# KorAP/Datok

Measured on AMD Instinct MI355X. Metric: input MB/s tokenized, tokenizer_de.matok, higher is better.
Workload: dtype u32 table cells, u8 symbol codes; 1 GPU; tokenizer_de.matok, 4096 equal-length 4096 B synthetic German docs per batch (BASELINE.json configs[1]); table_layout=matrix: state-major fused u32 cells, docs_per_gpu=4096, doc_bytes=4096, parallelism=documents sharded over 1 GPU(s), no data-path collective, batches_in_flight=3, inputs=one per batch in flight (generator seeds 2, 3, 4 on rank 0)

## Files before the change

datok_amd/_lib.py:

```python
import ctypes as C
import os
import subprocess

_HERE = os.path.dirname(os.path.abspath(__file__))
LIB_PATH = os.environ.get("DATOK_GPU_LIB") or os.path.join(_HERE, "libdatok_gpu.so")

OK, E_IO, E_FORMAT, E_NO_DEVICE, E_HIP, E_ARG, E_MODEL, E_CAPACITY, E_STATE, E_NOMEM = 0, -1, -2, -3, -4, -5, -6, -7, -8, -9
ST_WINDOW_OVERFLOW, ST_EMPTY_TEXT, ST_BAD_MODEL, ST_IRREGULAR, ST_STEP_LIMIT, ST_INTERNAL = 1, 2, 4, 8, 16, 32
ST_BAD_OFFSET = 64

EXPORTS = [
    "dtk_device_count", "dtk_set_device", "dtk_strerror", "dtk_last_hip_error",
    "dtk_model_load", "dtk_model_load_mem", "dtk_model_free", "dtk_model_type", "dtk_model_get_info",
    "dtk_model_info_mem",
    "dtk_batch_create", "dtk_batch_free", "dtk_batch_set_input", "dtk_batch_set_input_device",
    "dtk_batch_run", "dtk_batch_sync", "dtk_batch_stream", "dtk_batch_totals",
    "dtk_batch_set_profiling", "dtk_batch_stage_ms", "dtk_batch_set_chunking", "dtk_batch_set_warm_extend",
    "dtk_batch_result_device", "dtk_batch_result_host", "dtk_transduce", "dtk_free",
    "dtk_foma_to_matok", "dtk_foma_to_datok", "dtk_transduce_replay", "dtk_batch_render_device", "dtk_batch_render_host",
    "dtk_batch_status_host", "dtk_transduce_release", "dtk_transduce_result",
    "dtk_pipeline_create", "dtk_pipeline_free", "dtk_pipeline_set_chunking", "dtk_pipeline_run",
    "dtk_pinned_alloc", "dtk_pinned_free",
    "dtk_batch_set_result_fields", "dtk_batch_download_begin", "dtk_pipeline_set_result_fields",
    "dtk_batch_set_download_stream", "dtk_batch_download_stream", "dtk_batch_done", "dtk_batch_set_streams",
    "dtk_debug_configure",
    "dtk_multi_create", "dtk_multi_free", "dtk_multi_type", "dtk_multi_set_result_fields", "dtk_multi_set_chunking", "dtk_multi_run",
]


class ModelInfo(C.Structure):
    _fields_ = [("kind", C.c_int32), ("epsilon", C.c_int32), ("unknown", C.c_int32),
                ("identity", C.c_int32), ("final_state", C.c_int32), ("sigma_count", C.c_int32),
                ("state_count", C.c_uint32), ("array_len", C.c_uint64),
                ("n_eps_states", C.c_uint32), ("max_eps_chain", C.c_uint32),
                ("entry_bytes", C.c_uint32), ("device_bytes", C.c_uint64),
                ("unknown_used", C.c_uint32), ("dense_states", C.c_uint32),
                ("stream_codes", C.c_uint32)]


class Totals(C.Structure):
    _fields_ = [("n_docs", C.c_uint32), ("n_bytes", C.c_uint64), ("n_tokens", C.c_uint64),
                ("n_sent", C.c_uint64), ("n_texts", C.c_uint64), ("n_flagged", C.c_uint64),
                ("walk_steps", C.c_uint64), ("n_lanes", C.c_uint32), ("chunk_bytes", C.c_uint32),
                ("repair_rounds", C.c_uint32)]


class ResultView(C.Structure):
    _fields_ = [("tok_off", C.c_void_p), ("sent_off", C.c_void_p), ("text_off", C.c_void_p),
# ... 95 lines not shown
    L.dtk_foma_to_matok.restype = C.c_int
    L.dtk_foma_to_datok.argtypes = [vp, C.c_size_t, C.POINTER(vp), C.POINTER(C.c_size_t)]
    L.dtk_foma_to_datok.restype = C.c_int
    L.dtk_free.argtypes = [vp]
    L.dtk_free.restype = None
    L.dtk_pipeline_create.argtypes = [u64, u32, u32, C.POINTER(vp)]
    L.dtk_pipeline_free.argtypes = [vp]
    L.dtk_pipeline_free.restype = None
    L.dtk_pipeline_set_chunking.argtypes = [vp, u32, u32]
    L.dtk_pipeline_run.argtypes = [vp, vp, vp, vp, u32, u32, SLICE_FN, vp]
    L.dtk_multi_create.argtypes = [C.c_char_p, C.POINTER(C.c_int), u32, u64, u32, u32, C.POINTER(vp)]
    L.dtk_multi_free.argtypes = [vp]
    L.dtk_multi_free.restype = None
    L.dtk_multi_type.argtypes = [vp]
    L.dtk_multi_type.restype = C.c_char_p
    L.dtk_multi_set_result_fields.argtypes = [vp, u32]
    L.dtk_multi_set_chunking.argtypes = [vp, u32, u32]
    L.dtk_multi_run.argtypes = [vp, vp, vp, u32, u32, SLICE_FN, vp]
    L.dtk_pinned_alloc.restype = vp
    L.dtk_pinned_alloc.argtypes = [sz]
    L.dtk_pinned_free.argtypes = [vp]
    L.dtk_pinned_free.restype = None
    L.dtk_debug_configure.argtypes = [C.c_char_p, C.c_char_p]
    for k, v in os.environ.items():
        if k.startswith("DATOK_") and k not in ("DATOK_GPU_LIB", "DATOK_GATHER_TIMEOUT"):
            L.dtk_debug_configure(k.encode(), v.encode())
    _lib = L
    return L


def check(code, what=""):
    if code != OK:
        raise DatokGpuError(code, what)
```

datok_amd/csrc/dtk_batch.cpp:

```cpp
#include <algorithm>
#include <cstdio>
#include <cstring>

#include "dtk_host.h"

int pin_fit(dtk_batch::PinBuf &pb, size_t n) {
  if (n <= pb.cap && pb.p) return DTK_OK;
  if (pb.p) HIP_TRY(hipHostFree(pb.p));
  pb.p = nullptr; pb.cap = 0;
  const size_t cap = std::max<size_t>(n + n / 4, 256);
  HIP_TRY(hipHostMalloc(&pb.p, cap, hipHostMallocDefault));
  pb.cap = cap;
  return DTK_OK;
}

static int alloc_outputs(dtk_batch *b, uint64_t tok, uint64_t sent, uint64_t text) {
  auto grow = [&](auto *&p, uint64_t n) -> int {
    if (p) HIP_TRY(hipFree(p));
    p = nullptr;
    HIP_TRY(hipMalloc((void **)&p, std::max<uint64_t>(n, 4) * 4));
    return DTK_OK;
  };
  int rc;
  if (tok > b->tok_cap) {
// ... 23 lines not shown
  if (dtk_device_count() <= 0) return DTK_E_NO_DEVICE;
  dtk_batch *b = new dtk_batch();
  b->max_bytes = max_bytes;
  b->max_docs = max_docs;
  auto fail = [&](int rc) { dtk_batch_free(b); return rc; };
#define B_TRY(call)                                                  \
  do {                                                               \
    hipError_t e_ = (call);                                          \
    if (e_ != hipSuccess) return fail(hip_fail(e_, #call));          \
  } while (0)
  B_TRY(hipGetDevice(&b->device));
  B_TRY(hipStreamCreateWithFlags(&b->stream, hipStreamNonBlocking));
  if (g_dbg.round_limit >= 0) b->round_limit = (uint32_t)g_dbg.round_limit;
  const uint64_t pad = 256;
  B_TRY(hipMalloc((void **)&b->d_text_own, max_bytes + pad));
  B_TRY(hipMalloc((void **)&b->d_off_own, ((uint64_t)max_docs + 1) * 8));
  B_TRY(hipMalloc((void **)&b->d_sym, (max_bytes + pad) * 2));
  B_TRY(hipMalloc((void **)&b->d_rsbits, (max_bytes + pad) / 8 + 64));
  B_TRY(hipMalloc((void **)&b->d_bits, (EVB_KINDS * ((max_bytes + max_docs) / 32 + 8) + 8) * 4));
  b->acc_bytes = DTK_TOTALS_BYTES + 3 * ((uint64_t)max_docs + 1) * 8 + 4 * (uint64_t)max_docs * 4 + 64;
  B_TRY(hipMalloc((void **)&b->d_acc, b->acc_bytes));
  B_TRY(hipMalloc((void **)&b->d_redo, (uint64_t)max_docs * 4));
  B_TRY(hipMalloc((void **)&b->d_blk_doc, (max_bytes / DTK_SYM_BLOCK_BYTES + 3) * 4));

  B_TRY(hipMalloc((void **)&b->d_chunk_off, ((uint64_t)max_docs + 1) * 4));
  B_TRY(hipMalloc((void **)&b->d_big_docs, ((uint64_t)max_docs + 1) * 4));
  B_TRY(hipMalloc((void **)&b->d_csr, 3 * ((uint64_t)max_docs + 1) * 8));
  b->d_tok_off = b->d_csr; b->d_sent_off = b->d_csr + ((uint64_t)max_docs + 1); b->d_text_off = b->d_csr + 2 * ((uint64_t)max_docs + 1);
  B_TRY(hipMalloc((void **)&b->d_doc_ns, ((uint64_t)max_docs + 1) * 4));
  B_TRY(hipMalloc((void **)&b->d_scan_ws, ((uint64_t)max_docs / 2048 + 2) * 4 * 8));
  B_TRY(hipMalloc((void **)&b->d_out_off, ((uint64_t)max_docs + 1) * 8));

  B_TRY(hipHostMalloc((void **)&b->h_totals, DTK_TOTALS_BYTES, hipHostMallocDefault));
  B_TRY(hipHostMalloc((void **)&b->h_off_pin, ((uint64_t)max_docs + 1) * 8, hipHostMallocDefault));
#undef B_TRY
  int rc = alloc_outputs(b, max_bytes / 3 + max_docs + 16, max_bytes / 8 + 2ull * max_docs + 16,
                         max_bytes / 64 + 2ull * max_docs + 16);
  if (rc != DTK_OK) return fail(rc);
  *out = b;
  return DTK_OK;
}

extern "C" void dtk_batch_free(dtk_batch *b) {
  if (!b) return;
  if (b->stream) (void)hipStreamSynchronize(b->stream);
  if (b->up_stream) (void)hipStreamSynchronize(b->up_stream);
  if (b->ev_up) (void)hipEventDestroy(b->ev_up);
  if (b->dl_begun && !b->dl_waited) (void)hipEventSynchronize(b->ev_dl);
  if (b->dl_stream && b->dl_own) (void)hipStreamDestroy(b->dl_stream);
  if (b->ev_ran) (void)hipEventDestroy(b->ev_ran);
  if (b->ev_dl) (void)hipEventDestroy(b->ev_dl);
  for (auto &pb : b->pin)
    if (pb.p) (void)hipHostFree(pb.p);
  if (b->h_plan.p) (void)hipHostFree(b->h_plan.p);
  void *ptrs[] = {b->d_text_own, b->d_off_own, b->d_sym, b->d_rsbits, b->d_bits, b->d_acc, b->d_redo, b->d_chunk_off, b->d_blk_doc, b->d_big_docs,
                  b->d_lane_doc, b->d_lane_cnt, b->d_lane_start, b->d_lane_end, b->d_lane_plan,
                  b->d_seg_tab, b->d_seg_sum, b->d_seg_in,
                  b->d_csr, b->d_rstart, b->d_rend, b->d_sent,
                  b->d_bstart, b->d_bend, b->d_ttok, b->d_tsent,
                  b->d_sbefore, b->d_ts_end, b->d_doc_ns, b->d_scan_ws, b->d_rws, b->d_out_off, b->d_out,
                  b->d_exact_ids, b->d_exact_cnt, b->d_exact_off, b->d_calls, b->d_r16};
  for (void *p : ptrs)
    if (p) (void)hipFree(p);
  if (b->h_totals) (void)hipHostFree(b->h_totals);
  if (b->h_off_pin) (void)hipHostFree(b->h_off_pin);
  for (hipEvent_t e : b->ev)
    if (e) (void)hipEventDestroy(e);
  if (b->stream && b->stream_own) (void)hipStreamDestroy(b->stream);
  delete b;
}

extern "C" void *dtk_batch_stream(dtk_batch *b) { return b ? (void *)b->stream : nullptr; }

static int wait_ran(dtk_batch *b) {
  if (b->stream_own) HIP_TRY(hipStreamSynchronize(b->stream));
  else if (b->ev_ran_valid) HIP_TRY(hipEventSynchronize(b->ev_ran));
  return DTK_OK;
}
// ... 310 lines not shown
    b->d_tok_off = b->d_csr; b->d_sent_off = b->d_csr + (nd + 1); b->d_text_off = b->d_csr + 2 * (nd + 1);
    b->d_totals = (uint64_t *)q; q += DTK_TOTALS_BYTES;
    b->d_tok_cnt = (uint64_t *)q; q += (nd + 1) * 8;
    b->d_sent_cnt = (uint64_t *)q; q += (nd + 1) * 8;
    b->d_text_cnt = (uint64_t *)q; q += (nd + 1) * 8;
    b->d_status = (uint32_t *)q; q += nd * 4;
    b->d_first_bad = (uint32_t *)q; q += nd * 4;
    b->d_fail_lane = (uint32_t *)q; q += nd * 4;
    b->d_doc_tail = (uint32_t *)q; q += nd * 4;
    const size_t acc_used = ((size_t)(q - b->d_acc) + 15) & ~(size_t)15;
    b->bit_words = (uint32_t)(((b->total + nd) / 32 + 8) & ~(uint64_t)3);
    const bool fold = b->total > 0;
    fold_acc = fold && b->acc_primed && acc_used / 16 < 0xFFFFFFFFull && !g_dbg.clear_kernel;
    if (!fold_acc) {
      if (dtk_launch_clear2(b->d_acc, acc_used, b->d_bits, fold ? 0 : (size_t)EVB_KINDS * b->bit_words * 4, s))
        return hip_fail(hipGetLastError(), "clear");
      b->acc_primed = true;
    }
    acc_bytes = acc_used;
  }
  STAGE(1);
  if (dtk_launch_symbolize(b->d_text, b->d_off, b->n_docs, b->total, &m->sig, b->d_sym,
                           b->d_text == b->d_text_own, b->d_blk_doc, (unsigned long long *)(b->d_totals + 6), b->d_rsbits,
                           b->d_bits, b->bit_words, fold_acc ? b->d_acc : nullptr, acc_bytes, ++b->epoch, s))
    return hip_fail(hipGetLastError(), "symbolize");
  STAGE(2);
  DtkWalkArgs w = walk_args(b);
  bool fix_in_scan = false;
  DtkSpecArgs sp_first{};
  if (b->chunk == 0) {
    STAGE(3); STAGE(4);
    if (dtk_launch_walk(&m->tab, &w, s)) return hip_fail(hipGetLastError(), "walk");
    STAGE(5); STAGE(6); STAGE(7);
  } else {
    DtkSpecArgs sp = spec_args(b, false);
    sp_first = sp;
    uint32_t *nb = (uint32_t *)(b->d_totals + 8);
    const bool split = g_dbg.split_start != 0 || sp.lds_words == 0;
    b->dev_rounds = g_dbg.dev_rounds >= 0 ? (uint32_t)g_dbg.dev_rounds : (b->expect_repairs ? 2u : 0u);
    if (b->dev_rounds > 3u) b->dev_rounds = 3u;
    fix_in_scan = b->n_docs <= 8192u && b->dev_rounds == 0;
#define SPEC(stage)                                                                               \
  do {                                                                                            \
    if (dtk_launch_spec(&m->tab, &w, &sp, stage, cmp_mask_of(m), b->d_redo, nb, s))               \
      return hip_fail(hipGetLastError(), "speculative walk");                                     \
  } while (0)
    if (split) {
// ... 51 lines not shown
  if (e != hipSuccess) (void)hipGetLastError();
  return e == hipSuccess ? 1 : 0;
}

extern "C" int dtk_batch_set_profiling(dtk_batch *b, int enable) {
  if (!b) return DTK_E_ARG;
  if (enable && !b->ev[0])
    for (auto &e : b->ev) HIP_TRY(hipEventCreate(&e));
  b->profiling = enable != 0;
  return DTK_OK;
}

extern "C" int dtk_batch_stage_ms(dtk_batch *b, float ms[DTK_N_STAGES]) {
  if (!b || !ms) return DTK_E_ARG;
  if (!b->ran || !b->profiling) return DTK_E_STATE;
  HIP_TRY(hipStreamSynchronize(b->stream));
  for (int i = 0; i < DTK_N_STAGES; i++) HIP_TRY(hipEventElapsedTime(&ms[i], b->ev[i], b->ev[i + 1]));
  return DTK_OK;
}

extern "C" int dtk_batch_sync(dtk_batch *b) {
  if (!b) return DTK_E_ARG;
  return wait_own(b);
}

static int run_exact(dtk_batch *b) {
  const dtk_model *m = b->last_model;
  hipStream_t s = b->stream;
  const uint32_t nd = b->n_docs;
  std::vector<uint32_t> st(nd);
  HIP_TRY(hipMemcpy(st.data(), b->d_status, (size_t)nd * 4, hipMemcpyDeviceToHost));
  for (uint32_t d = 0; d < nd; d++)
    if (st[d] & ST_IRREGULAR) b->h_exact_ids.push_back(d);
  const uint32_t n = (uint32_t)b->h_exact_ids.size();
  if (n == 0) return DTK_OK;
  if (n > b->exact_cap) {
    void *old[] = {b->d_exact_ids, b->d_exact_cnt, b->d_exact_off};
    for (void *p : old)
      if (p) HIP_TRY(hipFree(p));
    b->d_exact_ids = b->d_exact_cnt = nullptr; b->d_exact_off = nullptr; b->exact_cap = 0;
    const uint64_t cap = (uint64_t)n + n / 4 + 16;
    HIP_TRY(hipMalloc((void **)&b->d_exact_ids, cap * 4));
    HIP_TRY(hipMalloc((void **)&b->d_exact_cnt, cap * 4));
    HIP_TRY(hipMalloc((void **)&b->d_exact_off, (cap + 1) * 8));
    b->exact_cap = (uint32_t)cap;
  }
// ... 161 lines not shown
```

datok_amd/csrc/dtk_host.h:

```cpp
#pragma once
#include <hip/hip_runtime.h>

#include <string>
#include <type_traits>
#include <vector>

#include "../../include/datok_gpu.h"
#include "dtk_internal.h"

#pragma GCC visibility push(hidden)


int hip_fail(hipError_t e, const char *what);
#define HIP_TRY(call)                                   \
  do {                                                  \
    hipError_t e_ = (call);                             \
    if (e_ != hipSuccess) return hip_fail(e_, #call);   \
  } while (0)

struct DtkDebug {
  int sym16 = 0;
  int force_wide = 0;
  int file_columns = 0;
  int no_fused = 0;
  int wide_fused = 0;
  int no_dense = 0;
  int small_max = -1;
  int lds_bits = 1;
  int split_start = 0;
  int dev_rounds = -1;
  int compact_full = 0;
  int clear_kernel = 0;
  int round_limit = -1;
  int debug_repair = 0;
};
extern DtkDebug g_dbg;


struct dtk_model {
  int kind = 0;
  int epsilon = 0, unknown = 0, identity = 0, final_state = 0, sigma_count = 0;
  uint32_t state_count = 0;
  std::vector<uint16_t> col;
  uint32_t dense_states = 0;
  uint64_t array_len = 0;
  uint32_t n_eps_states = 0, max_eps_chain = 0, unknown_used = 0;
  uint64_t device_bytes = 0;
  int device = 0;
  bool host_only = false;
  std::vector<uint32_t> sigma_runes;
  std::vector<uint16_t> sigma_syms;
  uint16_t ascii[256];
  void *d_tab = nullptr;
  uint16_t *d_ascii = nullptr;
  uint32_t *d_runes = nullptr;
  uint16_t *d_syms = nullptr;
  void *d_codes = nullptr;
// ... 22 lines not shown
  uint16_t *d_sym = nullptr;
  uint32_t *d_rsbits = nullptr;
  uint32_t *d_bits = nullptr;
  uint32_t bit_words = 0;
  uint32_t *d_doc_tail = nullptr;
  uint8_t *d_acc = nullptr;
  uint64_t acc_bytes = 0;
  uint32_t *d_status = nullptr;
  std::vector<uint64_t> h_doc_off;
  uint32_t cfg_chunk = 0xFFFFFFFFu;
  uint32_t cfg_extend = 240;
  uint32_t cfg_warm = 8;
  uint32_t chunk = 0;
  bool plan_valid = false;
  uint32_t n_lanes = 0, lane_cap = 0;
  uint32_t *d_lane_doc = nullptr, *d_chunk_off = nullptr, *d_redo = nullptr;
  uint32_t *d_seg_tab = nullptr;
  DtkSegSum *d_seg_sum = nullptr;
  DtkSegIn *d_seg_in = nullptr;
  uint32_t n_segs = 0, seg_cap = 0;
  bool long_docs = false;
  uint32_t max_doc_lanes = 0;
  uint32_t *d_blk_doc = nullptr;
  uint32_t small_max = 0, n_big = 0;
  uint32_t *d_big_docs = nullptr;
  uint32_t *d_first_bad = nullptr, *d_fail_lane = nullptr;
  DtkLaneCount *d_lane_cnt = nullptr;
  DtkLaneState *d_lane_start = nullptr, *d_lane_end = nullptr;
  DtkLanePlan *d_lane_plan = nullptr;
  uint32_t repair_rounds = 0;
  const dtk_model *last_model = nullptr;
  uint32_t last_flags = 0;
  uint64_t *d_csr = nullptr;
  uint64_t *d_tok_off = nullptr, *d_sent_off = nullptr, *d_text_off = nullptr;
  uint64_t *d_tok_cnt = nullptr, *d_sent_cnt = nullptr, *d_text_cnt = nullptr;
  uint64_t *d_scan_ws = nullptr;
  uint64_t *d_totals = nullptr;
  uint32_t dev_rounds = 0;
  bool expect_repairs = false;
  uint32_t round_limit = 0xFFFFFFFFu;
  bool acc_primed = false;
  uint64_t epoch = 0;
  bool expect_eot = false;
  bool ran_full = false;
  uint64_t *h_totals = nullptr;
  uint64_t *h_off_pin = nullptr;
// ... 80 lines not shown
```

datok_amd/csrc/dtk_internal.h:

```cpp
#pragma once
#include <stddef.h>
#include <stdint.h>

#define DTK_FIRSTBIT 0x80000000u
#define DTK_SECONDBIT 0x40000000u
#define DTK_RESTBIT 0x3fffffffu
#define DTK_EOT 4u
#define DTK_WINDOW 1024u
#define DTK_WINDOW_BYTES 4104u

#define DTK_SYM_MASK 0x7FFu
#define DTK_SYM_MAX 2047u
#define DTK_SYM_W_SHIFT 11
#define DTK_SYM_CLS_SHIFT 14
#define DTK_SYM_WIDTH(e) (((uint32_t)(e) >> DTK_SYM_W_SHIFT) & 7u)
#define DTK_SYM_IS_START(e) (DTK_SYM_WIDTH(e) != 0u)
#define DTK_WIN 32u
#define DTK_WIN_ROW 36u
#define DTK_SYM_CONT 0xFFu
#ifndef DTK_WIN8
#define DTK_WIN8 32u
#endif
struct DtkSym {
  const void *base;
// ... 213 lines not shown

#define DTK_TOHOST_MAX 14
struct DtkToHostArgs {
  const void *src[DTK_TOHOST_MAX];
  void *dst[DTK_TOHOST_MAX];
  uint64_t bytes[DTK_TOHOST_MAX];
  int32_t count_from[DTK_TOHOST_MAX];
  uint64_t cap[DTK_TOHOST_MAX];
  uint32_t n;
  const uint64_t *totals;
  const uint32_t *skip_if;
  uint64_t *done;
  uint64_t epoch;
};

#ifdef __cplusplus
extern "C" {
#endif
int dtk_launch_to_host(const struct DtkToHostArgs *args, void *stream);
int dtk_launch_pack_r16(const int32_t *rs, const int32_t *re, uint32_t *out, uint64_t n, void *stream);
int dtk_launch_symbolize(const uint8_t *text, const uint64_t *doc_off, uint32_t n_docs,
                         uint64_t total, const struct DtkSigmaDev *sig, void *sym, int padded,
                         const uint32_t *blk_doc, unsigned long long *n_invalid, uint32_t *rs_bits,
                         uint32_t *ev_bits, uint32_t bit_words, void *acc, uint64_t acc_bytes, uint64_t epoch, void *stream);
#ifndef DTK_SYM_BLOCK_BYTES
#define DTK_SYM_BLOCK_BYTES 4096u
#endif
int dtk_launch_walk(const struct DtkTableDev *tab, const struct DtkWalkArgs *args, void *stream);
int dtk_launch_spec(const struct DtkTableDev *tab, const struct DtkWalkArgs *args,
                    const struct DtkSpecArgs *spec, int stage, uint32_t cmp_mask, uint32_t *redo_out,
                    uint32_t *n_bad, void *stream);
int dtk_launch_spec_check(const struct DtkWalkArgs *args, const struct DtkSpecArgs *spec, int stage, uint32_t cmp_mask,
                          uint32_t *redo_out, uint32_t *n_bad, void *stream);
int dtk_launch_redo_clear(const struct DtkWalkArgs *args, const struct DtkSpecArgs *spec, void *stream);
int dtk_launch_compact(const struct DtkCompactArgs *args, uint32_t small_max, const uint32_t *big_docs, uint32_t n_big,
                       int which, void *stream);
int dtk_launch_exact(const struct DtkTableDev *tab, const struct DtkExactArgs *args, void *stream);
int dtk_launch_seg_prepare(const struct DtkCompactArgs *args, const uint32_t *doc_seg0, void *stream);
int dtk_launch_render(const struct DtkRenderArgs *args, int stage, void *stream);
uint32_t dtk_render_tiles(uint64_t n);
int dtk_launch_clear2(void *a, uint64_t a_bytes, void *b, uint64_t b_bytes, void *stream);
int dtk_launch_scan3(const uint64_t *ca, const uint64_t *cb, const uint64_t *cc, uint64_t *a, uint64_t *b,
                     uint64_t *c, uint32_t n_docs, uint64_t *totals, const uint32_t *status, uint64_t *ws,
                     const struct DtkSpecArgs *fix_spec, uint32_t *redo_out, uint32_t *n_bad, const uint32_t *skip_if,
                     void *stream);
#ifdef __cplusplus
}
// ... 2 lines not shown
```

datok_amd/csrc/dtk_model.cpp:

```cpp
#include <zlib.h>

#include <algorithm>
#include <cstdio>
#include <cstdlib>
#include <cstring>

#include "dtk_host.h"


static thread_local std::string g_hip_err;

int hip_fail(hipError_t e, const char *what) {
  g_hip_err = std::string(what) + ": " + hipGetErrorString(e);
  return e == hipErrorNoDevice || e == hipErrorInvalidDevice ? DTK_E_NO_DEVICE : DTK_E_HIP;
}

extern "C" const char *dtk_last_hip_error(void) { return g_hip_err.c_str(); }

extern "C" const char *dtk_strerror(int code) {
  switch (code) {
    case DTK_OK: return "ok";
    case DTK_E_IO: return "cannot open or read the tokenizer file";
    case DTK_E_FORMAT: return "not a gzip'd MATOK/DATOK file (magic, version or length)";
    case DTK_E_NO_DEVICE: return "no usable HIP device (this library has no CPU path)";
// ... 10 lines not shown
extern "C" int dtk_device_count(void) {
  int n = 0;
  if (hipGetDeviceCount(&n) != hipSuccess) return 0;
  return n;
}

extern "C" int dtk_set_device(int device) {
  HIP_TRY(hipSetDevice(device));
  return DTK_OK;
}

DtkDebug g_dbg;

extern "C" int dtk_debug_configure(const char *key, const char *value) {
  if (!key) return DTK_E_ARG;
  const int v = value ? atoi(value) : 1;
  const struct { const char *name; int *field; bool flag; } tab[] = {
      {"SYM16", &g_dbg.sym16, true}, {"FORCE_WIDE", &g_dbg.force_wide, true}, {"FILE_COLUMNS", &g_dbg.file_columns, true},
      {"NO_FUSED", &g_dbg.no_fused, true}, {"WIDE_FUSED", &g_dbg.wide_fused, true}, {"NO_DENSE", &g_dbg.no_dense, true}, {"SMALL_MAX", &g_dbg.small_max, false},
      {"LDS_BITS", &g_dbg.lds_bits, false}, {"SPLIT_START", &g_dbg.split_start, false}, {"DEV_ROUNDS", &g_dbg.dev_rounds, false},
      {"COMPACT_FULL", &g_dbg.compact_full, true}, {"CLEAR_KERNEL", &g_dbg.clear_kernel, true},
      {"ROUND_LIMIT", &g_dbg.round_limit, false}, {"DEBUG_REPAIR", &g_dbg.debug_repair, true}};
  if (strncmp(key, "DATOK_", 6) == 0) key += 6;
  for (const auto &e : tab)
    if (strcmp(key, e.name) == 0) {
      *e.field = e.flag ? ((value && value[0] == '0' && value[1] == 0) ? 0 : 1) : v;
      return DTK_OK;
    }
  return DTK_E_ARG;
}


int go_decode_host(const uint8_t *p, size_t n, uint32_t *r) {
  *r = 0xFFFD;
  if (n == 0) return 0;
  uint32_t b0 = p[0];
  if (b0 < 0x80) { *r = b0; return 1; }
  if (b0 < 0xC2 || b0 > 0xF4) return 1;
  if (b0 < 0xE0) {
    if (n < 2 || (p[1] & 0xC0) != 0x80) return 1;
    *r = ((b0 & 0x1F) << 6) | (p[1] & 0x3F);
    return 2;
  }
  if (b0 < 0xF0) {
    uint32_t lo = b0 == 0xE0 ? 0xA0 : 0x80, hi = b0 == 0xED ? 0x9F : 0xBF;
    if (n < 3 || p[1] < lo || p[1] > hi || (p[2] & 0xC0) != 0x80) return 1;
// ... 514 lines not shown
```

datok_amd/csrc/dtk_symbolize.hip:

```cpp
#include "dtk_device.h"


__device__ __forceinline__ uint32_t go_width(uint32_t b0, uint32_t b1, uint32_t b2, uint32_t b3, uint32_t avail) {
  const uint32_t c1 = (b1 & 0xC0u) == 0x80u, c2 = (b2 & 0xC0u) == 0x80u, c3 = (b3 & 0xC0u) == 0x80u;
  const uint32_t two = (uint32_t)(b0 - 0xC2u < 0x1Eu) & (uint32_t)(avail >= 2u) & c1;
  const uint32_t lo3 = b0 == 0xE0u ? 0xA0u : 0x80u, hi3 = b0 == 0xEDu ? 0x9Fu : 0xBFu;
  const uint32_t three = (uint32_t)((b0 & 0xF0u) == 0xE0u) & (uint32_t)(avail >= 3u) & (uint32_t)(b1 >= lo3) &
                         (uint32_t)(b1 <= hi3) & c2;
  const uint32_t lo4 = b0 == 0xF0u ? 0x90u : 0x80u, hi4 = b0 == 0xF4u ? 0x8Fu : 0xBFu;
  const uint32_t four = (uint32_t)(b0 - 0xF0u <= 4u) & (uint32_t)(avail >= 4u) & (uint32_t)(b1 >= lo4) &
                        (uint32_t)(b1 <= hi4) & c2 & c3;
  return 1u + two + 2u * three + 3u * four;
}


#define SYM_BLOCK_BYTES DTK_SYM_BLOCK_BYTES
#define SYM_TILE 512u
#define SYM_SIG_LDS 64u
#define SYM_HALF 1024u
#define SYM_THREADS (WAVE * (SYM_BLOCK_BYTES / SYM_HALF))
#define SYM_DOFF (SYM_BLOCK_BYTES / 16u)

template <bool ALIGNED4, bool SYM8>
__global__ __launch_bounds__(SYM_THREADS) void k_symbolize(const uint8_t *__restrict__ text,
                                                    const uint64_t *__restrict__ doc_off,
                                                    uint32_t n_docs, uint64_t total, DtkSigmaDev sig,
                                                    void *__restrict__ sym_,
                                                    const uint32_t *__restrict__ blk_doc,
                                                    unsigned long long *__restrict__ n_invalid,
                                                    uint32_t *__restrict__ rs_bits,
                                                    uint32_t *__restrict__ ev_bits, uint32_t bit_words,
                                                    uint4 *__restrict__ acc, uint32_t acc16,
                                                    unsigned long long epoch) {
  if (acc) {
    const uint4 z = make_uint4(0u, 0u, 0u, 0u);
    for (uint32_t i = blockIdx.x * SYM_THREADS + threadIdx.x; i < acc16; i += gridDim.x * SYM_THREADS) {
      if (i == 3u) reinterpret_cast<unsigned long long *>(acc)[7] = 0ull;
      else acc[i] = z;
    }
  }
  uint16_t *__restrict__ sym = static_cast<uint16_t *>(sym_);
  uint8_t *__restrict__ sym8 = static_cast<uint8_t *>(sym_);
  __shared__ uint32_t s_rs[SYM_BLOCK_BYTES / 32];
  __shared__ uint16_t lut[128];
  __shared__ uint16_t lat[256];
  __shared__ uint32_t s_runes[SYM_SIG_LDS];
  __shared__ uint16_t s_syms[SYM_SIG_LDS];
  __shared__ uint32_t s_txt[SYM_BLOCK_BYTES / 4 + 4];
  __shared__ uint16_t s_qs[SYM_BLOCK_BYTES / SYM_HALF][SYM_HALF];
  __shared__ uint64_t s_doff[SYM_DOFF];
  const uint32_t tid = threadIdx.x, lane = tid & (WAVE - 1u), half = tid >> 6;
  uint16_t *s_q = s_qs[half];
  const bool sig_lds = sig.n_runes <= SYM_SIG_LDS;
  for (uint32_t i = tid; i < SYM_BLOCK_BYTES / 32; i += SYM_THREADS) s_rs[i] = 0;
  for (uint32_t i = tid; i < 256u; i += SYM_THREADS) {
    if (SYM8) {
      lat[i] = sig.code_lt256[i];
      if (sig_lds && i < sig.n_runes) { s_runes[i] = sig.runes[i]; s_syms[i] = sig.code_runes[i]; }
    } else {
      const uint32_t e = (sig.ascii[i] & DTK_SYM_MASK) | (i == DTK_EOT ? (1u << DTK_SYM_CLS_SHIFT) : 0u);
      lat[i] = (uint16_t)e;
      if (i < 128u) lut[i] = (uint16_t)(e | (1u << DTK_SYM_W_SHIFT));
      if (sig_lds && i < sig.n_runes) { s_runes[i] = sig.runes[i]; s_syms[i] = sig.syms[i]; }
    }
  }
  const uint64_t block_start = (uint64_t)blockIdx.x * SYM_BLOCK_BYTES;
  const uint32_t n_here = (uint32_t)min((uint64_t)SYM_BLOCK_BYTES, total - block_start);
  const uint32_t d_lo = blk_doc[blockIdx.x];
  const uint32_t d_hi = min(blk_doc[blockIdx.x + 1], n_docs - 1);
  const uint32_t n_off = d_hi - d_lo + 2u;
  if (n_off <= SYM_DOFF && tid < n_off) s_doff[tid] = doc_off[d_lo + tid];
  {
    auto load4 = [&](uint64_t g) -> uint32_t {
      if (ALIGNED4) return g < total ? *reinterpret_cast<const uint32_t *>(text + g) : 0u;
      uint32_t x = 0;
      for (int k = 0; k < 4; k++)
        if (g + k < total) x |= (uint32_t)text[g + k] << (8 * k);
      return x;
    };
    uint32_t v[SYM_BLOCK_BYTES / 4 / SYM_THREADS];
#pragma unroll
    for (uint32_t r = 0; r < SYM_BLOCK_BYTES / 4 / SYM_THREADS; r++) v[r] = load4(block_start + (r * SYM_THREADS + tid) * 4u);
    uint32_t halo = 0;
    if (tid == 0 && block_start >= 4) halo = load4(block_start - 4);
    if (tid == 1) halo = load4(block_start + SYM_BLOCK_BYTES);
#pragma unroll
    for (uint32_t r = 0; r < SYM_BLOCK_BYTES / 4 / SYM_THREADS; r++) s_txt[1 + r * SYM_THREADS + tid] = v[r];
    if (tid == 0) s_txt[0] = halo;
    if (tid == 1) s_txt[1 + SYM_BLOCK_BYTES / 4] = halo;
  }
  __syncthreads();
  const uint8_t *__restrict__ sb = reinterpret_cast<const uint8_t *>(s_txt) + 4;

  const uint64_t lo_start = doc_off[d_lo], lo_end = doc_off[d_lo + 1];
  if (ev_bits) {
    const uint64_t ga = block_start + d_lo, gb = block_start + n_here + d_hi + 1u;
    const uint32_t wa = blockIdx.x == 0 ? 0u : (uint32_t)(ga >> 5);
    uint32_t wb = (uint32_t)((gb + 31u) >> 5);
    if (wb > bit_words || blockIdx.x == gridDim.x - 1) wb = bit_words;
    for (uint32_t w = wa + tid; w < wb; w += SYM_THREADS)
#pragma unroll
      for (uint32_t k = 0; k < EVB_KINDS; k++) ev_bits[(size_t)k * bit_words + w] = 0u;
  }
  const bool sym16 = ((reinterpret_cast<uintptr_t>(sym_) + (SYM8 ? 1ull : 2ull) * block_start) & (SYM8 ? 7u : 15u)) == 0;

  if (half * SYM_HALF < n_here) {
    uint32_t qn = 0;
    auto light = [&](auto full_tag, uint32_t it) {
      constexpr bool FULL = decltype(full_tag)::value;
      const uint32_t i0 = half * SYM_HALF + it * SYM_TILE + lane * 8u;
      const uint32_t w0 = s_txt[1 + (i0 >> 2)], w1 = s_txt[2 + (i0 >> 2)];
      uint32_t left = 8u;
      if (!FULL) left = i0 < n_here ? (n_here - i0 >= 8u ? 8u : n_here - i0) : 0u;
      if (SYM8) {
        if (FULL || (left == 8u && sym16)) {
          *reinterpret_cast<uint2 *>(sym8 + block_start + i0) = make_uint2(w0, w1);
        } else {
          for (uint32_t j = 0; j < left; j++) sym8[block_start + i0 + j] = (uint8_t)((j < 4u ? w0 >> (8u * j) : w1 >> (8u * j - 32u)));
        }
      } else {
        const uint32_t e0 = lut[w0 & 0x7Fu], e1 = lut[(w0 >> 8) & 0x7Fu];
        const uint32_t e2 = lut[(w0 >> 16) & 0x7Fu], e3 = lut[(w0 >> 24) & 0x7Fu];
        const uint32_t e4 = lut[w1 & 0x7Fu], e5 = lut[(w1 >> 8) & 0x7Fu];
        const uint32_t e6 = lut[(w1 >> 16) & 0x7Fu], e7 = lut[(w1 >> 24) & 0x7Fu];
        if (FULL || (left == 8u && sym16)) {
          *reinterpret_cast<uint4 *>(sym + block_start + i0) =
// ... 95 lines not shown
            if (r < rune) l = m + 1; else h = m - 1;
          }
        }
        if (SYM8) sym8[g] = (uint8_t)(start ? a_cls : DTK_SYM_CONT);
        else sym[g] = (uint16_t)(a_cls | (start ? wd << DTK_SYM_W_SHIFT : 0u));
        if (start) atomicOr(&s_rs[pos >> 5], 1u << (pos & 31u));
        bad = start && wd == 1u;
      }
      if (__ballot(bad) != 0ull && lane == 0 &&
          __hip_atomic_load(n_invalid, __ATOMIC_RELAXED, __HIP_MEMORY_SCOPE_AGENT) != epoch)
        atomicMax(n_invalid, epoch);
    }
  }
  __syncthreads();
  for (uint32_t i = tid; i < SYM_BLOCK_BYTES / 32; i += SYM_THREADS)
    if (i * 32u < n_here) rs_bits[(block_start >> 5) + i] = s_rs[i];
}


extern "C" int dtk_launch_symbolize(const uint8_t *text, const uint64_t *doc_off, uint32_t n_docs,
                                    uint64_t total, const DtkSigmaDev *sig, void *sym, int padded,
                                    const uint32_t *blk_doc, unsigned long long *n_invalid, uint32_t *rs_bits,
                                    uint32_t *ev_bits, uint32_t bit_words, void *acc, uint64_t acc_bytes,
                                    uint64_t epoch, void *stream) {
  if (total == 0 || n_docs == 0) return 0;
  const uint32_t blocks = (uint32_t)((total + SYM_BLOCK_BYTES - 1) / SYM_BLOCK_BYTES);
  const bool al4 = (((uintptr_t)text) & 3u) == 0 && (padded || (total & 3u) == 0);
  auto go = [&](auto k) {
    hipLaunchKernelGGL(k, dim3(blocks), dim3(SYM_THREADS), 0, (hipStream_t)stream, text, doc_off, n_docs,
                       total, *sig, sym, blk_doc, n_invalid, rs_bits, ev_bits, bit_words, (uint4 *)acc, (uint32_t)(acc_bytes / 16),
                       (unsigned long long)epoch);
  };
  if (sig->n_codes) { if (al4) go(k_symbolize<true, true>); else go(k_symbolize<false, true>); }
  else { if (al4) go(k_symbolize<true, false>); else go(k_symbolize<false, false>); }
  return (int)hipGetLastError();
}
```

datok_amd/host.py:

```python
import ctypes as C
import io
import sys

import numpy as np

from . import _lib
from ._lib import ModelInfo, RenderView, ResultView, Totals, check, lib

TOKENS, SENTENCES, TOKEN_POS, SENTENCE_POS, NEWLINE_AFTER_EOT = 1, 2, 4, 8, 16
SIMPLE = TOKENS | SENTENCES
OFFSETS_ONLY, NO_BYTE_OFFSETS, NO_RUNE_OFFSETS = 256, 512, 1024

EV_S_EOT, EV_E_EOT, EV_TOK_END, EV_S_EPS, EV_S_EOF, EV_E_EOF = 1, 2, 4, 8, 32, 64
EVB_END, EVB_START, EVB_SEPS, EVB_TEOT, EVB_SEOT = 0, 1, 2, 3, 4


def _decode_runes(b: bytes):
    out, i, n = [], 0, len(b)
    while i < n:
        b0 = b[i]
        r, w = 0xFFFD, 1
        if b0 < 0x80:
            r = b0
        elif 0xC2 <= b0 < 0xE0:
# ... 310 lines not shown

    AUTO_CHUNK = 0xFFFFFFFF

    def set_chunking(self, chunk_bytes=AUTO_CHUNK, warm_bytes=8, extend=None):
        check(lib().dtk_batch_set_chunking(self._h, int(chunk_bytes), int(warm_bytes)), "dtk_batch_set_chunking")
        if extend is not None:
            check(lib().dtk_batch_set_warm_extend(self._h, int(extend)), "dtk_batch_set_warm_extend")

    def set_profiling(self, enable=True):
        check(lib().dtk_batch_set_profiling(self._h, int(bool(enable))), "dtk_batch_set_profiling")

    STAGES = ("clear", "symbolize", "spec_start", "spec_link", "walk", "spec_verify", "spec_fix", "scan", "compact")

    def stage_ms(self):
        ms = (C.c_float * 9)()
        check(lib().dtk_batch_stage_ms(self._h, C.byref(ms)), "dtk_batch_stage_ms")
        return dict(zip(self.STAGES, [float(x) for x in ms]))

    def totals(self):
        t = Totals()
        check(lib().dtk_batch_totals(self._h, C.byref(t)), "dtk_batch_totals")
        return {k: getattr(t, k) for k, _ in Totals._fields_}

    def result_device(self) -> ResultView:
        v = ResultView()
        check(lib().dtk_batch_result_device(self._h, C.byref(v)), "dtk_batch_result_device")
        return v

    def render_device(self, flags=SIMPLE) -> RenderView:
        v = RenderView()
        check(lib().dtk_batch_render_device(self._h, flags, C.byref(v)), "dtk_batch_render_device")
        return v

    def render(self, flags=SIMPLE):
        v = RenderView()
        check(lib().dtk_batch_render_host(self._h, flags, C.byref(v)), "dtk_batch_render_host")
        off = np.frombuffer((C.c_char * ((self.n_docs + 1) * 8)).from_address(v.doc_off), dtype=np.uint64).copy()
        data = C.string_at(v.bytes, v.total) if v.total else b""
        return data, off

    R_CSR, R_TOK_RUNE, R_TOK_BYTE, R_SENT, R_TEXTS, R_STATUS, R_EVENTS, R_ALL = 1, 2, 4, 8, 16, 32, 64, 127
    R_TOK_RUNE16 = 128
    R_EAGER = 256

    def set_result_fields(self, fields=R_ALL):
        check(lib().dtk_batch_set_result_fields(self._h, int(fields)), "dtk_batch_set_result_fields")
# ... 176 lines not shown
```

include/datok_gpu.h:

```cpp
#ifndef DATOK_GPU_H
#define DATOK_GPU_H

#include <stddef.h>
#include <stdint.h>

#ifdef __cplusplus
extern "C" {
#endif

enum {
  DTK_OK = 0,
  DTK_E_IO = -1,
  DTK_E_FORMAT = -2,
  DTK_E_NO_DEVICE = -3,
  DTK_E_HIP = -4,
  DTK_E_ARG = -5,
  DTK_E_MODEL = -6,
  DTK_E_CAPACITY = -7,
  DTK_E_STATE = -8,
  DTK_E_NOMEM = -9
};

enum {
  DTK_TOKENS = 1,
// ... 6 lines not shown
  DTK_NO_BYTE_OFFSETS = 512,
  DTK_NO_RUNE_OFFSETS = 1024
};

enum {
  DTK_ST_WINDOW_OVERFLOW = 1,
  DTK_ST_EMPTY_TEXT = 2,
  DTK_ST_BAD_MODEL = 4,
  DTK_ST_IRREGULAR = 8,
  DTK_ST_STEP_LIMIT = 16,
  DTK_ST_INTERNAL = 32,
  DTK_ST_BAD_OFFSET = 64
};

typedef struct dtk_model dtk_model;
typedef struct dtk_batch dtk_batch;

int dtk_device_count(void);
int dtk_set_device(int device);
const char *dtk_strerror(int code);
const char *dtk_last_hip_error(void);

int dtk_debug_configure(const char *key, const char *value);

int dtk_model_load(const char *path, dtk_model **out);
int dtk_model_load_mem(const void *gz_bytes, size_t n, dtk_model **out);
void dtk_model_free(dtk_model *m);
int dtk_foma_to_matok(const void *gz_bytes, size_t n, void **out, size_t *out_n);
int dtk_foma_to_datok(const void *gz_bytes, size_t n, void **out, size_t *out_n);
const char *dtk_model_type(const dtk_model *m);

typedef struct {
  int32_t kind;
  int32_t epsilon, unknown, identity, final_state, sigma_count;
  uint32_t state_count;
  uint64_t array_len;
  uint32_t n_eps_states;
  uint32_t max_eps_chain;
  uint32_t entry_bytes;
  uint64_t device_bytes;
  uint32_t unknown_used;
  uint32_t dense_states;
  uint32_t stream_codes;
} dtk_model_info;
int dtk_model_get_info(const dtk_model *m, dtk_model_info *out);
int dtk_model_info_mem(const void *gz_bytes, size_t n, dtk_model_info *out);
// ... 127 lines not shown
```

Baseline: 171,600 MB/s.

## Add SWAR register fast path for fully valid UTF-8 symbolize blocks

Adds a fast path to the symbolize kernel for full, aligned, single-byte-code blocks. It classifies UTF-8 bytes with SWAR bit tricks on 16-byte register vectors, taking neighbour words from adjacent lanes via DPP. When the block has no invalid sequences it writes the rune-start bits and symbol codes straight from registers, skipping the LDS staging path. Latin-1 two-byte runes use a table lookup and other multi-byte runes use a binary search. Invalid blocks fall back to the old path, and a debug env var, a per-block flag array and a debug export exist to compare the two paths.

```diff
diff --git a/datok_amd/_lib.py b/datok_amd/_lib.py
--- a/datok_amd/_lib.py
+++ b/datok_amd/_lib.py
@@ -23,7 +23,7 @@
     "dtk_pinned_alloc", "dtk_pinned_free",
     "dtk_batch_set_result_fields", "dtk_batch_download_begin", "dtk_pipeline_set_result_fields",
     "dtk_batch_set_download_stream", "dtk_batch_download_stream", "dtk_batch_done", "dtk_batch_set_streams",
-    "dtk_debug_configure",
+    "dtk_debug_configure", "dtk_batch_debug_stream",
     "dtk_multi_create", "dtk_multi_free", "dtk_multi_type", "dtk_multi_set_result_fields", "dtk_multi_set_chunking", "dtk_multi_run",
 ]
 
@@ -165,6 +165,7 @@
     L.dtk_pinned_free.argtypes = [vp]
     L.dtk_pinned_free.restype = None
     L.dtk_debug_configure.argtypes = [C.c_char_p, C.c_char_p]
+    L.dtk_batch_debug_stream.argtypes = [vp, vp, u64, vp, u64, C.POINTER(u32), C.POINTER(u64)]
     for k, v in os.environ.items():
         if k.startswith("DATOK_") and k not in ("DATOK_GPU_LIB", "DATOK_GATHER_TIMEOUT"):
             L.dtk_debug_configure(k.encode(), v.encode())
diff --git a/datok_amd/csrc/dtk_batch.cpp b/datok_amd/csrc/dtk_batch.cpp
--- a/datok_amd/csrc/dtk_batch.cpp
+++ b/datok_amd/csrc/dtk_batch.cpp
@@ -69,6 +69,7 @@
   B_TRY(hipMalloc((void **)&b->d_acc, b->acc_bytes));
   B_TRY(hipMalloc((void **)&b->d_redo, (uint64_t)max_docs * 4));
   B_TRY(hipMalloc((void **)&b->d_blk_doc, (max_bytes / DTK_SYM_BLOCK_BYTES + 3) * 4));
+  B_TRY(hipMalloc((void **)&b->d_blk_old, (max_bytes / DTK_SYM_BLOCK_BYTES + 3) * 4));
 
   B_TRY(hipMalloc((void **)&b->d_chunk_off, ((uint64_t)max_docs + 1) * 4));
   B_TRY(hipMalloc((void **)&b->d_big_docs, ((uint64_t)max_docs + 1) * 4));
@@ -100,7 +101,7 @@
   for (auto &pb : b->pin)
     if (pb.p) (void)hipHostFree(pb.p);
   if (b->h_plan.p) (void)hipHostFree(b->h_plan.p);
-  void *ptrs[] = {b->d_text_own, b->d_off_own, b->d_sym, b->d_rsbits, b->d_bits, b->d_acc, b->d_redo, b->d_chunk_off, b->d_blk_doc, b->d_big_docs,
+  void *ptrs[] = {b->d_text_own, b->d_off_own, b->d_sym, b->d_rsbits, b->d_bits, b->d_acc, b->d_redo, b->d_chunk_off, b->d_blk_doc, b->d_blk_old, b->d_big_docs,
                   b->d_lane_doc, b->d_lane_cnt, b->d_lane_start, b->d_lane_end, b->d_lane_plan,
                   b->d_seg_tab, b->d_seg_sum, b->d_seg_in,
                   b->d_csr, b->d_rstart, b->d_rend, b->d_sent,
@@ -457,7 +458,8 @@
   STAGE(1);
   if (dtk_launch_symbolize(b->d_text, b->d_off, b->n_docs, b->total, &m->sig, b->d_sym,
                            b->d_text == b->d_text_own, b->d_blk_doc, (unsigned long long *)(b->d_totals + 6), b->d_rsbits,
-                           b->d_bits, b->bit_words, fold_acc ? b->d_acc : nullptr, acc_bytes, ++b->epoch, s))
+                           b->d_bits, b->bit_words, fold_acc ? b->d_acc : nullptr, acc_bytes, ++b->epoch,
+                           b->d_blk_old, g_dbg.sym_path_old, s))
     return hip_fail(hipGetLastError(), "symbolize");
   STAGE(2);
   DtkWalkArgs w = walk_args(b);
@@ -555,6 +557,26 @@
 extern "C" int dtk_batch_sync(dtk_batch *b) {
   if (!b) return DTK_E_ARG;
   return wait_own(b);
+}
+
+extern "C" int dtk_batch_debug_stream(dtk_batch *b, void *stream_out, uint64_t stream_cap, uint32_t *rs_out,
+                                      uint64_t rs_cap, uint32_t *entry_bytes, uint64_t *n_old) {
+  if (!b || !stream_out || !rs_out || !entry_bytes || !n_old) return DTK_E_ARG;
+  if (!b->ran || !b->last_model) return DTK_E_STATE;
+  const int rc = wait_own(b);
+  if (rc != DTK_OK) return rc;
+  const uint32_t eb = b->last_model->sig.n_codes ? 1u : 2u;
+  const uint64_t rs_words = (b->total + 31) / 32, nblk = (b->total + DTK_SYM_BLOCK_BYTES - 1) / DTK_SYM_BLOCK_BYTES;
+  if (stream_cap < b->total * eb || rs_cap < rs_words) return DTK_E_ARG;
+  *entry_bytes = eb;
+  *n_old = 0;
+  if (b->total == 0) return DTK_OK;
+  std::vector<uint32_t> old((size_t)nblk);
+  HIP_TRY(hipMemcpy(stream_out, b->d_sym, (size_t)(b->total * eb), hipMemcpyDeviceToHost));
+  HIP_TRY(hipMemcpy(rs_out, b->d_rsbits, (size_t)rs_words * 4, hipMemcpyDeviceToHost));
+  HIP_TRY(hipMemcpy(old.data(), b->d_blk_old, (size_t)nblk * 4, hipMemcpyDeviceToHost));
+  for (uint32_t o : old) *n_old += o != 0;
+  return DTK_OK;
 }
 
 static int run_exact(dtk_batch *b) {
diff --git a/datok_amd/csrc/dtk_host.h b/datok_amd/csrc/dtk_host.h
--- a/datok_amd/csrc/dtk_host.h
+++ b/datok_amd/csrc/dtk_host.h
@@ -33,6 +33,7 @@
   int clear_kernel = 0;
   int round_limit = -1;
   int debug_repair = 0;
+  int sym_path_old = 0;
 };
 extern DtkDebug g_dbg;
 
@@ -101,6 +102,7 @@
   bool long_docs = false;
   uint32_t max_doc_lanes = 0;
   uint32_t *d_blk_doc = nullptr;
+  uint32_t *d_blk_old = nullptr;
   uint32_t small_max = 0, n_big = 0;
   uint32_t *d_big_docs = nullptr;
   uint32_t *d_first_bad = nullptr, *d_fail_lane = nullptr;
diff --git a/datok_amd/csrc/dtk_internal.h b/datok_amd/csrc/dtk_internal.h
--- a/datok_amd/csrc/dtk_internal.h
+++ b/datok_amd/csrc/dtk_internal.h
@@ -259,7 +259,8 @@
 int dtk_launch_symbolize(const uint8_t *text, const uint64_t *doc_off, uint32_t n_docs,
                          uint64_t total, const struct DtkSigmaDev *sig, void *sym, int padded,
                          const uint32_t *blk_doc, unsigned long long *n_invalid, uint32_t *rs_bits,
-                         uint32_t *ev_bits, uint32_t bit_words, void *acc, uint64_t acc_bytes, uint64_t epoch, void *stream);
+                         uint32_t *ev_bits, uint32_t bit_words, void *acc, uint64_t acc_bytes, uint64_t epoch,
+                         uint32_t *blk_old, int path_old, void *stream);
 #ifndef DTK_SYM_BLOCK_BYTES
 #define DTK_SYM_BLOCK_BYTES 4096u
 #endif
diff --git a/datok_amd/csrc/dtk_model.cpp b/datok_amd/csrc/dtk_model.cpp
--- a/datok_amd/csrc/dtk_model.cpp
+++ b/datok_amd/csrc/dtk_model.cpp
@@ -56,6 +56,12 @@
       {"COMPACT_FULL", &g_dbg.compact_full, true}, {"CLEAR_KERNEL", &g_dbg.clear_kernel, true},
       {"ROUND_LIMIT", &g_dbg.round_limit, false}, {"DEBUG_REPAIR", &g_dbg.debug_repair, true}};
   if (strncmp(key, "DATOK_", 6) == 0) key += 6;
+  if (strcmp(key, "SYM_PATH") == 0) {
+    const bool old = value && strcmp(value, "old") == 0;
+    if (!old && !(value && strcmp(value, "auto") == 0)) return DTK_E_ARG;
+    g_dbg.sym_path_old = old;
+    return DTK_OK;
+  }
   for (const auto &e : tab)
     if (strcmp(key, e.name) == 0) {
       *e.field = e.flag ? ((value && value[0] == '0' && value[1] == 0) ? 0 : 1) : v;
diff --git a/datok_amd/csrc/dtk_symbolize.hip b/datok_amd/csrc/dtk_symbolize.hip
--- a/datok_amd/csrc/dtk_symbolize.hip
+++ b/datok_amd/csrc/dtk_symbolize.hip
@@ -21,6 +21,34 @@
 #define SYM_THREADS (WAVE * (SYM_BLOCK_BYTES / SYM_HALF))
 #define SYM_DOFF (SYM_BLOCK_BYTES / 16u)
 
+struct SymMarks { uint32_t cont, lead2, lead3, other, latin; };
+__device__ __forceinline__ SymMarks sym_marks(uint32_t w) {
+  const uint32_t h = w & 0x80808080u;
+  const uint32_t c0 = (w << 1) & h;
+  const uint32_t e0 = (w << 2) & c0;
+  const uint32_t f0 = (w << 3) & e0;
+  SymMarks m;
+  m.cont = h ^ c0;
+  const uint32_t cx = c0 ^ e0;
+  const uint32_t v = w & 0x1E1E1E1Eu;
+  m.lead2 = cx & (v + 0x7E7E7E7Eu);
+  m.latin = m.lead2 & ~(v + 0x7C7C7C7Cu);
+  m.lead3 = e0 ^ f0;
+  m.other = f0 | (cx ^ m.lead2);
+  return m;
+}
+__device__ __forceinline__ void sym_marks_e0d(uint32_t w, SymMarks &m) {
+  const uint32_t e0d = m.lead3 & ~(((w & 0x0F0F0F0Fu) + 0x7F7F7F7Fu) & (((w ^ 0x0D0D0D0Du) & 0x0F0F0F0Fu) + 0x7F7F7F7Fu));
+  m.lead3 ^= e0d;
+  m.other |= e0d;
+}
+__device__ __forceinline__ uint32_t sym_up1(uint32_t x, uint32_t lo) { return __builtin_amdgcn_alignbit(x, lo, 24); }
+__device__ __forceinline__ uint32_t sym_marks8(uint32_t a, uint32_t b) {
+  const uint32_t m = (a >> 7) | (b >> 3);
+  return (m | (m >> 7) | (m >> 14) | (m >> 21)) & 0xFFu;
+}
+typedef uint32_t sym_u32x4 __attribute__((ext_vector_type(4), aligned(4)));
+
 template <bool ALIGNED4, bool SYM8>
 __global__ __launch_bounds__(SYM_THREADS) void k_symbolize(const uint8_t *__restrict__ text,
                                                     const uint64_t *__restrict__ doc_off,
@@ -31,7 +59,8 @@
                                                     uint32_t *__restrict__ rs_bits,
                                                     uint32_t *__restrict__ ev_bits, uint32_t bit_words,
                                                     uint4 *__restrict__ acc, uint32_t acc16,
-                                                    unsigned long long epoch) {
+                                                    unsigned long long epoch, uint32_t *__restrict__ blk_old,
+                                                    uint32_t path_old) {
   if (acc) {
     const uint4 z = make_uint4(0u, 0u, 0u, 0u);
     for (uint32_t i = blockIdx.x * SYM_THREADS + threadIdx.x; i < acc16; i += gridDim.x * SYM_THREADS) {
@@ -52,7 +81,6 @@
   const uint32_t tid = threadIdx.x, lane = tid & (WAVE - 1u), half = tid >> 6;
   uint16_t *s_q = s_qs[half];
   const bool sig_lds = sig.n_runes <= SYM_SIG_LDS;
-  for (uint32_t i = tid; i < SYM_BLOCK_BYTES / 32; i += SYM_THREADS) s_rs[i] = 0;
   for (uint32_t i = tid; i < 256u; i += SYM_THREADS) {
     if (SYM8) {
       lat[i] = sig.code_lt256[i];
@@ -68,6 +96,110 @@
   const uint32_t n_here = (uint32_t)min((uint64_t)SYM_BLOCK_BYTES, total - block_start);
   const uint32_t d_lo = blk_doc[blockIdx.x];
   const uint32_t d_hi = min(blk_doc[blockIdx.x + 1], n_docs - 1);
+  if (ev_bits) {
+    const uint64_t ga = block_start + d_lo, gb = block_start + n_here + d_hi + 1u;
+    const uint32_t wa = blockIdx.x == 0 ? 0u : (uint32_t)(ga >> 5);
+    uint32_t wb = (uint32_t)((gb + 31u) >> 5);
+    if (wb > bit_words || blockIdx.x == gridDim.x - 1) wb = bit_words;
+    for (uint32_t w = wa + tid; w < wb; w += SYM_THREADS)
+#pragma unroll
+      for (uint32_t k = 0; k < EVB_KINDS; k++) ev_bits[(size_t)k * bit_words + w] = 0u;
+  }
+
+  if (ALIGNED4 && SYM8 && !path_old && n_here == SYM_BLOCK_BYTES &&
+      ((reinterpret_cast<uintptr_t>(sym_) + block_start) & 15u) == 0) {
+    __shared__ uint32_t s_bad[SYM_THREADS / WAVE];
+    const uint64_t g0 = block_start + tid * 16u;
+    const sym_u32x4 v = *reinterpret_cast<const sym_u32x4 *>(text + g0);
+    uint32_t edge = 0u;
+    if (lane == 0u && g0 >= 4u) edge = *reinterpret_cast<const uint32_t *>(text + g0 - 4u);
+    if (lane == WAVE - 1u && g0 + 16u < total) {
+      edge = *reinterpret_cast<const uint32_t *>(text + g0 + 16u);
+      const uint64_t left = total - (g0 + 16u);
+      if (left < 4u) edge &= (1u << (8u * (uint32_t)left)) - 1u;
+    }
+    const uint32_t w0 = v.x, w1 = v.y, w2 = v.z, w3 = v.w;
+    const uint32_t wp = (uint32_t)__builtin_amdgcn_update_dpp((int)edge, (int)w3, 0x138, 0xF, 0xF, false);
+    const uint32_t wn = (uint32_t)__builtin_amdgcn_update_dpp((int)edge, (int)w0, 0x130, 0xF, 0xF, false);
+    SymMarks mp = sym_marks(wp), m0 = sym_marks(w0), m1 = sym_marks(w1), m2 = sym_marks(w2), m3 = sym_marks(w3);
+    if (mp.lead3 | m0.lead3 | m1.lead3 | m2.lead3 | m3.lead3) {
+      sym_marks_e0d(wp, mp); sym_marks_e0d(w0, m0); sym_marks_e0d(w1, m1); sym_marks_e0d(w2, m2); sym_marks_e0d(w3, m3);
+    }
+    const uint32_t cn = wn & ~(wn << 1) & 0x80808080u;
+    const uint32_t lp = mp.lead2 | mp.lead3, l0 = m0.lead2 | m0.lead3, l1 = m1.lead2 | m1.lead3, l2 = m2.lead2 | m2.lead3,
+                   l3 = m3.lead2 | m3.lead3;
+    const uint32_t tp = (mp.lead3 << 8) & mp.cont;
+    const uint32_t t0 = sym_up1(m0.lead3, mp.lead3) & m0.cont, t1 = sym_up1(m1.lead3, m0.lead3) & m1.cont,
+                   t2 = sym_up1(m2.lead3, m1.lead3) & m2.cont, t3 = sym_up1(m3.lead3, m2.lead3) & m3.cont;
+    const uint32_t tn = (m3.lead3 >> 24) & cn;
+    uint32_t bad = m0.other | m1.other | m2.other | m3.other;
+    bad |= ((sym_up1(l0, lp) | sym_up1(t0, tp)) ^ m0.cont) | ((sym_up1(l1, l0) | sym_up1(t1, t0)) ^ m1.cont) |
+           ((sym_up1(l2, l1) | sym_up1(t2, t1)) ^ m2.cont) | ((sym_up1(l3, l2) | sym_up1(t3, t2)) ^ m3.cont);
+    bad |= ((l3 >> 24) | sym_up1(tn, t3)) & 0x00008080u & ~cn;
+    for (uint32_t i = tid; i < d_hi - d_lo + 2u; i += SYM_THREADS) {
+      const uint64_t d = doc_off[d_lo + i];
+      if (d >= block_start && d < block_start + SYM_BLOCK_BYTES + 2u && d < total) bad |= (uint32_t)((text[d] & 0xC0u) == 0x80u);
+    }
+    const uint32_t wave_bad = __ballot(bad != 0u) != 0ull;
+    if (lane == 0u) s_bad[half] = wave_bad;
+    __syncthreads();
+    uint32_t block_bad = 0u;
+#pragma unroll
+    for (uint32_t k = 0; k < SYM_THREADS / WAVE; k++) block_bad |= s_bad[k];
+    if (!block_bad) {
+      if (blk_old && tid == 0u) blk_old[blockIdx.x] = 0u;
+      const uint32_t rs = ~(sym_marks8(m0.cont, m1.cont) | (sym_marks8(m2.cont, m3.cont) << 8)) & 0xFFFFu;
+      const uint32_t rs_hi = (uint32_t)__builtin_amdgcn_update_dpp(0, (int)rs, 0xF5, 0xF, 0xF, true);
+      if (!(lane & 1u)) rs_bits[(block_start >> 5) + (tid >> 1)] = rs | (rs_hi << 16);
+      static_assert(DTK_SYM_CONT == 0xFFu, "the continuation bytes are OR-ed into the code");
+      uint32_t o0 = w0 | (m0.cont - (m0.cont >> 7)), o1 = w1 | (m1.cont - (m1.cont >> 7)),
+               o2 = w2 | (m2.cont - (m2.cont >> 7)), o3 = w3 | (m3.cont - (m3.cont >> 7));
+      const uint32_t q0 = m0.latin, q1 = m1.latin, q2 = m2.latin, q3 = m3.latin;
+      auto latin = [&](uint32_t &q, uint32_t a, uint32_t b, uint32_t &o) {
+        const uint32_t sh = (uint32_t)__builtin_ctz(q | 0x80000000u) - 7u;
+        const uint32_t x = __builtin_amdgcn_alignbit(b, a, sh);
+        const uint32_t code = lat[(((x >> 8) & 0xFFu) + ((x & 1u) << 6)) & 0xFFu];
+        o ^= ((code ^ x) & ((q >> sh) & 0x80u ? 0xFFu : 0u)) << sh;
+        q &= q - 1u;
+      };
+      {
+        uint32_t a0 = q0, a1 = q1, a2 = q2, a3 = q3;
+        while (__builtin_amdgcn_ballot_w64((a0 | a1 | a2 | a3) != 0u) != 0ull) {
+          latin(a0, w0, w1, o0); latin(a1, w1, w2, o1); latin(a2, w2, w3, o2); latin(a3, w3, wn, o3);
+        }
+      }
+      uint32_t r0 = l0 ^ q0, r1 = l1 ^ q1, r2 = l2 ^ q2, r3 = l3 ^ q3;
+      while (__builtin_amdgcn_ballot_w64((r0 | r1 | r2 | r3) != 0u) != 0ull) {
+        if (r0 | r1 | r2 | r3) {
+          const uint32_t k = r0 ? 0u : (r1 ? 1u : (r2 ? 2u : 3u));
+          const uint32_t r = k == 0u ? r0 : (k == 1u ? r1 : (k == 2u ? r2 : r3));
+          const uint32_t a = k == 0u ? w0 : (k == 1u ? w1 : (k == 2u ? w2 : w3));
+          const uint32_t b = k == 0u ? w1 : (k == 1u ? w2 : (k == 2u ? w3 : wn));
+          const uint32_t sh = (uint32_t)__builtin_ctz(r) - 7u;
+          const uint32_t x = __builtin_amdgcn_alignbit(b, a, sh);
+          const uint32_t b0 = x & 0xFFu, b1 = (x >> 8) & 0xFFu, b2 = (x >> 16) & 0xFFu;
+          const bool three = b0 >= 0xE0u;
+          const uint32_t rune = three ? ((b0 & 0x0Fu) << 12) | ((b1 & 0x3Fu) << 6) | (b2 & 0x3Fu) : ((b0 & 0x1Fu) << 6) | (b1 & 0x3Fu);
+          uint32_t code = three ? sig.code_ident[3] : sig.code_ident[2];
+          int l = 0, h = (int)sig.n_runes - 1;
+          while (l <= h) {
+            const int m = (l + h) >> 1;
+            const uint32_t sr = sig_lds ? s_runes[m] : sig.runes[m];
+            if (sr == rune) { code = sig_lds ? (uint32_t)s_syms[m] : (uint32_t)sig.code_runes[m]; break; }
+            if (sr < rune) l = m + 1; else h = m - 1;
+          }
+          const uint32_t patch = ((code ^ b0) & 0xFFu) << sh;
+          o0 ^= k == 0u ? patch : 0u; o1 ^= k == 1u ? patch : 0u; o2 ^= k == 2u ? patch : 0u; o3 ^= k == 3u ? patch : 0u;
+          const uint32_t rest = r & (r - 1u);
+          r0 = k == 0u ? rest : r0; r1 = k == 1u ? rest : r1; r2 = k == 2u ? rest : r2; r3 = k == 3u ? rest : r3;
+        }
+      }
+      *reinterpret_cast<uint4 *>(sym8 + g0) = make_uint4(o0, o1, o2, o3);
+      return;
+    }
+  }
+  if (blk_old && tid == 0u) blk_old[blockIdx.x] = 1u;
+  for (uint32_t i = tid; i < SYM_BLOCK_BYTES / 32; i += SYM_THREADS) s_rs[i] = 0;
   const uint32_t n_off = d_hi - d_lo + 2u;
   if (n_off <= SYM_DOFF && tid < n_off) s_doff[tid] = doc_off[d_lo + tid];
   {
@@ -93,15 +225,6 @@
   const uint8_t *__restrict__ sb = reinterpret_cast<const uint8_t *>(s_txt) + 4;
 
   const uint64_t lo_start = doc_off[d_lo], lo_end = doc_off[d_lo + 1];
-  if (ev_bits) {
-    const uint64_t ga = block_start + d_lo, gb = block_start + n_here + d_hi + 1u;
-    const uint32_t wa = blockIdx.x == 0 ? 0u : (uint32_t)(ga >> 5);
-    uint32_t wb = (uint32_t)((gb + 31u) >> 5);
-    if (wb > bit_words || blockIdx.x == gridDim.x - 1) wb = bit_words;
-    for (uint32_t w = wa + tid; w < wb; w += SYM_THREADS)
-#pragma unroll
-      for (uint32_t k = 0; k < EVB_KINDS; k++) ev_bits[(size_t)k * bit_words + w] = 0u;
-  }
   const bool sym16 = ((reinterpret_cast<uintptr_t>(sym_) + (SYM8 ? 1ull : 2ull) * block_start) & (SYM8 ? 7u : 15u)) == 0;
 
   if (half * SYM_HALF < n_here) {
@@ -243,14 +366,14 @@
                                     uint64_t total, const DtkSigmaDev *sig, void *sym, int padded,
                                     const uint32_t *blk_doc, unsigned long long *n_invalid, uint32_t *rs_bits,
                                     uint32_t *ev_bits, uint32_t bit_words, void *acc, uint64_t acc_bytes,
-                                    uint64_t epoch, void *stream) {
+                                    uint64_t epoch, uint32_t *blk_old, int path_old, void *stream) {
   if (total == 0 || n_docs == 0) return 0;
   const uint32_t blocks = (uint32_t)((total + SYM_BLOCK_BYTES - 1) / SYM_BLOCK_BYTES);
   const bool al4 = (((uintptr_t)text) & 3u) == 0 && (padded || (total & 3u) == 0);
   auto go = [&](auto k) {
     hipLaunchKernelGGL(k, dim3(blocks), dim3(SYM_THREADS), 0, (hipStream_t)stream, text, doc_off, n_docs,
                        total, *sig, sym, blk_doc, n_invalid, rs_bits, ev_bits, bit_words, (uint4 *)acc, (uint32_t)(acc_bytes / 16),
-                       (unsigned long long)epoch);
+                       (unsigned long long)epoch, blk_old, (uint32_t)(path_old != 0));
   };
   if (sig->n_codes) { if (al4) go(k_symbolize<true, true>); else go(k_symbolize<false, true>); }
   else { if (al4) go(k_symbolize<true, false>); else go(k_symbolize<false, false>); }
diff --git a/datok_amd/host.py b/datok_amd/host.py
--- a/datok_amd/host.py
+++ b/datok_amd/host.py
@@ -356,6 +356,14 @@
         check(lib().dtk_batch_totals(self._h, C.byref(t)), "dtk_batch_totals")
         return {k: getattr(t, k) for k, _ in Totals._fields_}
 
+    def debug_stream(self):
+        eb, n_old = C.c_uint32(), C.c_uint64()
+        stream = np.zeros(2 * self.total, np.uint8)
+        rs = np.zeros((self.total + 31) // 32, np.uint32)
+        check(lib().dtk_batch_debug_stream(self._h, stream.ctypes.data, stream.nbytes, rs.ctypes.data, len(rs),
+                                           C.byref(eb), C.byref(n_old)), "dtk_batch_debug_stream")
+        return stream[:self.total * eb.value], rs, int(n_old.value)
+
     def result_device(self) -> ResultView:
         v = ResultView()
         check(lib().dtk_batch_result_device(self._h, C.byref(v)), "dtk_batch_result_device")
diff --git a/include/datok_gpu.h b/include/datok_gpu.h
--- a/include/datok_gpu.h
+++ b/include/datok_gpu.h
@@ -52,6 +52,8 @@
 const char *dtk_last_hip_error(void);
 
 int dtk_debug_configure(const char *key, const char *value);
+int dtk_batch_debug_stream(dtk_batch *b, void *stream_out, uint64_t stream_cap, uint32_t *rs_out, uint64_t rs_cap,
+                           uint32_t *entry_bytes, uint64_t *n_old);
 
 int dtk_model_load(const char *path, dtk_model **out);
 int dtk_model_load_mem(const void *gz_bytes, size_t n, dtk_model **out);
```

After: 178,800 MB/s, median of 6. +4.2%, better.
